# peterrum/deal-and-ceed-on-gpu

Hardware: AMD Instinct MI355X
Metric: BP5 DoFs/sec per CG iter (p=4, ~1e8 DoFs) + % HBM roofline at 1/2/4/8 GPUs (higher is better)
Workload: dtype f64

## Files before the change

### deal-and-ceed-on-gpu_amd/csrc/bp5_device.hip

```cpp
#include "bp5_device.hpp"


extern "C" int bp5_device_count(int *count)
{
  if (!count) return fail(BP5_ERR_INVALID, "null argument");
  int c = 0;
  hipError_t e = hipGetDeviceCount(&c);
  if (e != hipSuccess) { *count = 0; return fail(BP5_ERR_NO_DEVICE, hipGetErrorString(e)); }
  *count = c;
  return BP5_OK;
}
extern "C" int bp5_vec_alloc(size_t n, double **out)
{
  if (!out) return fail(BP5_ERR_INVALID, "null argument");
  HIP_TRY(hipMalloc((void **)out, std::max<size_t>(n, 1) * sizeof(double)));
  HIP_TRY(hipMemset(*out, 0, std::max<size_t>(n, 1) * sizeof(double)));
  HIP_TRY(hipStreamSynchronize(nullptr));
  return BP5_OK;
}
extern "C" int bp5_vec_free(double *v) { HIP_TRY(hipFree(v)); return BP5_OK; }
extern "C" int bp5_copy_h2d(void *dst, const void *src, size_t bytes) { HIP_TRY(hipMemcpy(dst, src, bytes, hipMemcpyHostToDevice)); return BP5_OK; }
extern "C" int bp5_copy_d2h(void *dst, const void *src, size_t bytes) { HIP_TRY(hipMemcpy(dst, src, bytes, hipMemcpyDeviceToHost)); return BP5_OK; }

static void tuning_from_environment(bp5_mf *mf);
// ... 120 lines not shown
    const uint32_t ns = mf->send_off.back();
    if (mf->recv_off.back() != d->n_ghost) { return fail(BP5_ERR_INVALID, "recv ranges must cover the ghost range"); }
    for (uint32_t s = 0; s < ns; ++s)
      if (d->send_indices_host[s] >= d->n_owned) { return fail(BP5_ERR_INVALID, "send index out of owned range"); }
    BP5_TRY(upload(&mf->d_send_idx, d->send_indices_host, ns));
    std::vector<uint8_t> sd(ns);
    for (uint32_t s = 0; s < ns; ++s) sd[s] = mf->h_constrained[d->send_indices_host[s]] ? 1 : 0;
    BP5_TRY(upload(&mf->d_send_dirichlet, sd.data(), sd.size()));
    HIP_TRY(hipMalloc((void **)&mf->d_sendbuf, std::max<size_t>(ns, 1) * sizeof(double)));
    HIP_TRY(hipMalloc((void **)&mf->d_recvbuf, std::max<size_t>(ns, 1) * sizeof(double)));
  } else if (d->n_ghost) { return fail(BP5_ERR_INVALID, "ghosts without a halo plan"); }
  HIP_TRY(hipMalloc((void **)&mf->d_partials, 8 * PARTIAL_STRIDE * sizeof(double)));
  HIP_TRY(hipMalloc((void **)&mf->d_sc, SC_COUNT * sizeof(double)));
  HIP_TRY(hipMalloc((void **)&mf->d_scalar, 8 * sizeof(double)));
  HIP_TRY(hipMalloc((void **)&mf->d_st, ST_COUNT * sizeof(int)));
  HIP_TRY(hipMemset(mf->d_sc, 0, SC_COUNT * sizeof(double)));
  HIP_TRY(hipMemset(mf->d_st, 0, ST_COUNT * sizeof(int)));
  HIP_TRY(hipStreamSynchronize(nullptr));
  HIP_TRY(hipHostMalloc((void **)&mf->h_sc, SC_COUNT * sizeof(double)));
  HIP_TRY(hipHostMalloc((void **)&mf->h_st, ST_COUNT * sizeof(int)));
  HIP_TRY(hipEventCreate(&mf->ev_solve[0]));
  HIP_TRY(hipEventCreate(&mf->ev_solve[1]));
  guard.m = nullptr;
  *out = mf;
  return BP5_OK;
}

extern "C" int bp5_mf_destroy(bp5_mf *mf)
{
  if (!mf) return BP5_OK;
  hipSetDevice(mf->device);
  hipStreamSynchronize(mf->stream);
  void *ptrs[] = {mf->d_constrained_bits, mf->d_l2g, mf->d_constrained, mf->d_send_idx, mf->d_coords, mf->d_tab, mf->d_tab_gauss, mf->d_l2g_padded,
                  mf->d_constraint_mask, mf->d_inv_jac, mf->d_JxW, mf->d_qpoints, mf->d_sendbuf, mf->d_recvbuf, mf->d_partials,
                  mf->d_sc, mf->d_scalar, mf->d_st, mf->ws_base, mf->d_stamps, mf->d_evec, mf->d_scalar_plane, mf->d_gcell, mf->d_hang_mask, mf->d_hang_I, mf->d_send_dirichlet, mf->d_signal, mf->ws_z, mf->wsc_base, mf->hc_base, mf->d_hc_off};
  for (void *p : ptrs) if (p) hipFree(p);
  if (mf->h_sc) hipHostFree(mf->h_sc);
  if (mf->h_st) hipHostFree(mf->h_st);
  for (hipEvent_t e : mf->ev_pool) hipEventDestroy(e);
  for (hipEvent_t e : mf->phase.ev) hipEventDestroy(e);
  for (hipEvent_t e : mf->ev_solve) if (e) hipEventDestroy(e);
  for (hipEvent_t e : mf->ev_halo) if (e) hipEventDestroy(e);
  for (hipEvent_t e : mf->ev_done) if (e) hipEventDestroy(e);
  if (mf->h_done) hipHostFree(mf->h_done);
  if (mf->comm_stream) { hipStreamSynchronize(mf->comm_stream); hipStreamDestroy(mf->comm_stream); }
  for (auto &kv : mf->march_plans) { hipFree(kv.second.team_off); hipFree(kv.second.entries); }
  for (auto &kv : mf->plans) {
    auto &q = kv.second;
    void *pp[] = {q.off, q.dofs, q.sh_dof, q.sh_off, q.sh_slot, q.pos, q.cell_round, q.team_rounds, q.partial, q.cell_off, q.pass_cell, q.pass_off, q.run_off, q.runs, q.gidx, q.packed, q.lattice, q.cell_pos, q.cr_start, q.cr_dof0, q.cr_soff, q.cr_slots, q.cr_tile};
    for (void *x : pp) if (x) hipFree(x);
// ... 1274 lines not shown
}
static void tuning_from_environment(bp5_mf *mf)
{
  mf->tune[BP5_TUNE_LATTICE_INDICES] = env_int("BP5_LATTICE_INDICES", 1) != 0;
  mf->tune[BP5_TUNE_EARLY_GATHER] = env_int("BP5_EARLY_GATHER", 1) != 0;
  mf->tune[BP5_TUNE_COMBINE_SIGNAL] = env_int("BP5_COMBINE_SIGNAL", 0) == 1;
  { const char *e = getenv("BP5_BOUNDARY_FIRST"); mf->tune[BP5_TUNE_BOUNDARY_FIRST] = !(e && !strcmp(e, "launches")); }
  mf->tune[BP5_TUNE_FOLD_SMALL] = env_int("BP5_FOLD_SMALL", 1) != 0;
  { const int u = env_int("BP5_UPDATE_UNROLL", 1); mf->tune[BP5_TUNE_UPDATE_UNROLL] = (u == 2 || u == 4) ? u : 1; }
  mf->tune[BP5_TUNE_UPDATE_FLAT] = env_int("BP5_UPDATE_FLAT", 1) != 0;
  { const int v = env_int("BP5_UPDATE_NT", -1); mf->tune[BP5_TUNE_UPDATE_NT] = v < 0 ? -1 : v != 0; }
  { const int v = env_int("BP5_COMBINE_WG_PER_CU", 16); mf->tune[BP5_TUNE_COMBINE_WG_PER_CU] = (v >= 0 && v <= 32) ? v : 16; }
  mf->tune[BP5_TUNE_INTERIOR_STORES] = env_int("BP5_INTERIOR_STORES", 1) != 0;
  mf->tune[BP5_TUNE_GHOST_COMBINE_ON_COMM] = env_int("BP5_GHOST_COMBINE_ON_COMM", 0) != 0;
  mf->tune[BP5_TUNE_FACE_CARRY] = env_int("BP5_FACE_CARRY", 1) != 0;
}
extern "C" int bp5_mf_set_tuning(bp5_mf *mf, int knob, int value)
{
  if (!mf || knob < 0 || knob >= BP5_TUNE_COUNT) return fail(BP5_ERR_INVALID, "unknown tuning knob");
  switch (knob) {
    case BP5_TUNE_UPDATE_UNROLL:
      if (value != 1 && value != 2 && value != 4) return fail(BP5_ERR_INVALID, "BP5_TUNE_UPDATE_UNROLL: 1, 2 or 4");
      break;
    case BP5_TUNE_UPDATE_NT:
      if (value < -1 || value > 1) return fail(BP5_ERR_INVALID, "BP5_TUNE_UPDATE_NT: -1, 0 or 1");
      break;
    case BP5_TUNE_COMBINE_WG_PER_CU:
      if (value < 0 || value > 32) return fail(BP5_ERR_INVALID, "BP5_TUNE_COMBINE_WG_PER_CU: 0 ... 32");
      break;
    case BP5_TUNE_LATTICE_INDICES:
      if (value != 0 && value != 1) return fail(BP5_ERR_INVALID, "switch: 0 or 1");
      if (value != mf->tune[knob] && mf->plans.count(-block_cpt(mf))) return fail(BP5_ERR_INVALID, "BP5_TUNE_LATTICE_INDICES: the block plan of this handle is already built");
      break;
    default:
      if (value != 0 && value != 1) return fail(BP5_ERR_INVALID, "switch: 0 or 1");
  }
  mf->tune[knob] = value;
  if (knob == BP5_TUNE_BOUNDARY_FIRST && mf->wait_value_ok >= 0) mf->can_wait_value = mf->wait_value_ok == 1 && value != 0;
  return BP5_OK;
}
extern "C" int bp5_mf_get_tuning(const bp5_mf *mf, int knob, int *value)
{
  if (!mf || !value || knob < 0 || knob >= BP5_TUNE_COUNT) return fail(BP5_ERR_INVALID, "unknown tuning knob");
  *value = mf->tune[knob];
// ... 74 lines not shown
  if (mf->overlap_now) HIP_TRY(hipEventRecord(mf->ev_halo[3], cs));
  return BP5_OK;
}
extern "C" int bp5_halo_scatter_add_start(bp5_mf *mf, double *v)
{
  if (!mf || !v) return fail(BP5_ERR_INVALID, "null argument");
  if (mf->neighbors.empty()) return BP5_OK;
  if (!mf->comm) return fail(BP5_ERR_INVALID, "halo exchange needs bp5_mf_set_comm");
  HIP_TRY(hipSetDevice(mf->device));
  BP5_TRY(halo_streams(mf));
  return scatter_exchange(mf, v, overlap_wanted(mf));
}
static int scatter_add_finish(bp5_mf *mf, double *v, FuseState *fuse)
{
  if (mf->overlap_now) HIP_TRY(hipStreamWaitEvent(mf->stream, mf->ev_halo[3], 0));
  for (size_t k = 0; k < mf->neighbors.size(); ++k) {
    const uint32_t sc = mf->send_off[k + 1] - mf->send_off[k];
    if (!sc) continue;
    if (fuse) {
      const uint32_t grid = std::min<uint32_t>((sc + 255) / 256, 1024u / (uint32_t)mf->neighbors.size());
      const uint32_t ng = fuse->ghosts_zeroed ? 0u : mf->n_ghost;
      hipLaunchKernelGGL(unpack_add_dots_kernel, dim3(grid), dim3(256), 0, mf->stream, mf->d_send_idx + mf->send_off[k],
                         mf->d_send_dirichlet + mf->send_off[k], sc, mf->d_recvbuf + mf->send_off[k], v, fuse->r, mf->d_partials,
                         fuse->n_cols, mf->d_st, v + mf->n_owned, const_cast<double *>(fuse->p) + mf->n_owned, ng);
      fuse->n_cols += grid;
      fuse->ghosts_zeroed = true;
    } else
      hipLaunchKernelGGL(unpack_add_kernel, dim3((sc + 255) / 256), dim3(256), 0, mf->stream, mf->d_send_idx + mf->send_off[k], sc,
                         mf->d_recvbuf + mf->send_off[k], v);
    KERNEL_CHECK();
  }
  if (fuse && fuse->ghosts_zeroed) return BP5_OK;
  return bp5_halo_zero_ghosts(mf, v);
}
extern "C" int bp5_halo_scatter_add_finish(bp5_mf *mf, double *v)
{
  if (!mf || !v) return fail(BP5_ERR_INVALID, "null argument");
  if (mf->neighbors.empty()) return BP5_OK;
  if (!mf->comm || !mf->comm_stream) return fail(BP5_ERR_INVALID, "bp5_halo_scatter_add_finish without bp5_halo_scatter_add_start");
  return scatter_add_finish(mf, v, nullptr);
}
// ... 324 lines not shown
  int mark(int k)
  {
    if (!on) return BP5_OK;
    if (used >= 4 * MAX_PROFILED) { on = false; return BP5_OK; }
    while ((size_t)used + 4 > mf->ev_pool.size()) { hipEvent_t e; HIP_TRY(hipEventCreate(&e)); mf->ev_pool.push_back(e); }
    HIP_TRY(hipEventRecord(mf->ev_pool[used + k], mf->stream));
    return BP5_OK;
  }
};

struct SolveState {
  ApplyProfile prof;
  int exchange = EXCHANGE_NONE;
  bool two_parts = false;
  bool gather_in_flight = false;
  bool dst_prezeroed = false, copies_dirichlet = false;
  bool phase_on = false;
  int phase_it = 0;
  uint8_t phase_recorded[bp5_mf::PhaseProfile::MAX_ITERS] = {};
};

static int phase_mark(bp5_mf *mf, SolveState &ss, int k)
{
  if (!ss.phase_on || ss.phase_it >= bp5_mf::PhaseProfile::MAX_ITERS) return BP5_OK;
  HIP_TRY(hipEventRecord(mf->phase.ev[(size_t)ss.phase_it * bp5_mf::PhaseProfile::MARKS + k], mf->stream));
  ss.phase_recorded[ss.phase_it] |= (uint8_t)(1u << k);
  return BP5_OK;
}

static int fused_unsplit(bp5_mf *mf, SolveState &ss, ApplyCall &call, const double *coef, const double *src, double *dst)
// ... 75 lines not shown
  BP5_TRY(phase_mark(mf, ss, 3));
  return scatter_add_finish(mf, dst, call.fuse);
}
static int fused_vmult_distributed(bp5_mf *mf, SolveState &ss, const double *coef, double *src, double *dst, const double *fuse_r, uint32_t *n_cols)
{
  if (ss.gather_in_flight) { ss.gather_in_flight = false; BP5_TRY(bp5_halo_gather_finish(mf, src)); }
  else {
    BP5_TRY(gather_start(mf, src, false));
    BP5_TRY(bp5_halo_gather_finish(mf, src));
  }
  BP5_TRY(phase_mark(mf, ss, 2));
  BP5_TRY(ss.prof.mark(0));
  BP5_TRY(ss.prof.mark(1));
  FuseState fuse;
  fuse.p = src; fuse.r = fuse_r;
  ApplyCall call;
  call.c0 = 0; call.c1 = mf->n_cells; call.overwrite = true;
  call.fuse = &fuse;
  call.exchange = ss.exchange;
  call.two_parts = ss.two_parts;
  if (ss.exchange == EXCHANGE_BOUNDARY_FIRST) BP5_TRY(fused_boundary_first(mf, ss, call, coef, src, dst));
  else if (ss.exchange == EXCHANGE_GHOST_ROWS_FIRST) BP5_TRY(fused_ghost_rows_first(mf, ss, call, coef, src, dst));
  else BP5_TRY(fused_unsplit(mf, ss, call, coef, src, dst));
  *n_cols = fuse.n_cols;
  if (!fuse.ghosts_zeroed) BP5_TRY(bp5_halo_zero_ghosts(mf, src));
  return BP5_OK;
}

static int solver_vmult(bp5_mf *mf, SolveState &ss, const double *coef, double *src, double *dst, bool zero, const double *fuse_r = nullptr,
                        uint32_t *n_cols = nullptr)
{
  ApplyProfile &prof = ss.prof;
  const bool dist = mf->has_neighbors();
  const bool fusing = n_cols != nullptr;
  if (dist && fusing) return fused_vmult_distributed(mf, ss, coef, src, dst, fuse_r, n_cols);
  ApplyCall call;
  call.c0 = 0; call.c1 = mf->n_cells;
  if (dist) {
    BP5_TRY(prof.mark(0));
// ... 281 lines not shown
  const int unroll = mf->tune[BP5_TUNE_UPDATE_UNROLL];
  const int gridu = stream_grid_flat(mf, n, 2 * unroll);
  const bool streaming = mf->tune[BP5_TUNE_UPDATE_NT] != 0;
  auto launch_update = [&](int mode) {
#define BP5_UPD(M, U, ZV, NT) hipLaunchKernelGGL((cgm_update_kernel<M, U, ZV, NT>), dim3(gridu), dim3(VB), 0, s, d, g, h, x, diag, n, mf->d_sc, mf->d_st)
#define BP5_UPD_U(M, ZV, NT) do { if (unroll == 1) BP5_UPD(M, 1, ZV, NT); else if (unroll == 2) BP5_UPD(M, 2, ZV, NT); else BP5_UPD(M, 4, ZV, NT); } while (0)
    if (mode == 0) { BP5_UPD_U(0, false, false); return; }
    if (prezero) { if (mode == 1) BP5_UPD_U(1, true, false); else BP5_UPD_U(2, true, false); return; }
    if (streaming) { if (mode == 1) BP5_UPD_U(1, false, true); else BP5_UPD_U(2, false, true); return; }
    if (mode == 1) BP5_UPD_U(1, false, false); else BP5_UPD_U(2, false, false);
#undef BP5_UPD_U
#undef BP5_UPD
  };
  const bool early_gather_enabled = mf->tune[BP5_TUNE_EARLY_GATHER] != 0;
  const bool early_gather = fused && dist_solve && early_gather_enabled;
  auto gather_under_update = [&](int mode) -> int {
    BP5_TRY(halo_streams(mf));
    const uint32_t ns = mf->send_off.back();
    if (ns) {
      const dim3 gr((ns + 255) / 256), bl(256);
      if (mode == 0) hipLaunchKernelGGL(cgm_pack_updated_kernel<0>, gr, bl, 0, s, mf->d_send_idx, ns, d, g, h, diag, mf->d_sc, mf->d_st, mf->d_sendbuf);
      else hipLaunchKernelGGL(cgm_pack_updated_kernel<1>, gr, bl, 0, s, mf->d_send_idx, ns, d, g, h, diag, mf->d_sc, mf->d_st, mf->d_sendbuf);
      KERNEL_CHECK();
    }
    return gather_exchange(mf, d, true);
  };
  int it = 1;
  for (; it <= prm->max_iter; ++it) {
    const int mode = it == 1 ? 0 : it % 2 == 0 ? 1 : 2;
    BP5_TRY(phase_mark(mf, ss, 0));
    if (early_gather) { BP5_TRY(gather_under_update(mode)); ss.gather_in_flight = true; }
    if (mode != 0) launch_update(mode);
    KERNEL_CHECK();
    BP5_TRY(phase_mark(mf, ss, 1));
    const bool one_launch = fused && !mf->comm;
    if (fused) {
      uint32_t n_cols = 0;
      BP5_TRY(vmult(d, h, g, &n_cols));
      BP5_TRY(phase_mark(mf, ss, 4));
      if (one_launch) hipLaunchKernelGGL(cgm_finalize4_kernel<true>, dim3(1), dim3(FIN4_THREADS), 0, s, mf->d_partials, (int)n_cols, mf->d_sc, mf->d_st);
      else hipLaunchKernelGGL(cgm_finalize4_kernel<false>, dim3(1), dim3(FIN4_THREADS), 0, s, mf->d_partials, (int)n_cols, mf->d_sc, mf->d_st);
    } else {
      BP5_TRY(vmult(d, h, nullptr, nullptr));
      BP5_TRY(phase_mark(mf, ss, 4));
      hipLaunchKernelGGL(cgm_dots_kernel, dim3(grid2), dim3(VB), 0, s, d, g, h, diag, n, mf->d_st, mf->d_partials,
                         fold_small ? (const uint32_t *)mf->d_constrained_bits : (const uint32_t *)nullptr);
      hipLaunchKernelGGL(finalize_kernel<7>, dim3(7), dim3(VB), 0, s, mf->d_partials, grid2, mf->d_sc + SC_R0, mf->d_st);
    }
    KERNEL_CHECK();
    BP5_TRY(phase_mark(mf, ss, 5));
    if (!one_launch) {
      BP5_TRY(bp5_comm_allreduce_sum(mf, mf->d_sc + SC_R0, 7));
      BP5_TRY(phase_mark(mf, ss, 6));
      hipLaunchKernelGGL(cgm_control_kernel, dim3(1), dim3(1), 0, s, mf->d_sc, mf->d_st);
      KERNEL_CHECK();
    } else
      BP5_TRY(phase_mark(mf, ss, 6));
    BP5_TRY(phase_mark(mf, ss, 7));
    if (ss.phase_on) ++ss.phase_it;
    if (check > 0 && it % check == 0 && it < prm->max_iter) {
      BP5_TRY(poll_state(mf));
      if (mf->h_st[ST_DONE]) break;
    }
  }
  if (prm->max_iter > 0) {
    launch_update(1);
    hipLaunchKernelGGL(cgm_control_kernel, dim3(1), dim3(1), 0, s, mf->d_sc, mf->d_st);
    KERNEL_CHECK();
  }
  const int status = solve_finish(mf, ss.prof, fused, op.schedule, !user, res);
// ... 742 lines not shown
```

### deal-and-ceed-on-gpu_amd/csrc/bp5_device.hpp

```cpp
#pragma once
#include "bp5_internal.hpp"
#include "bp5_kernels.hpp"

#include <hip/hip_runtime.h>
#include <rccl/rccl.h>

#include <algorithm>
#include <cmath>
#include <cstdio>
#include <cstdlib>
#include <cstring>
#include <map>
#include <memory>
#include <tuple>
#include <vector>

using namespace bp5;

#define HIP_TRY(expr)                                                                                              \
  do {                                                                                                             \
    hipError_t e_ = (expr);                                                                                        \
    if (e_ != hipSuccess)                                                                                          \
      return fail(e_ == hipErrorNoDevice || e_ == hipErrorInvalidDevice ? BP5_ERR_NO_DEVICE : BP5_ERR_HIP,         \
                  std::string(#expr) + ": " + hipGetErrorString(e_));                                              \
// ... 51 lines not shown
  uint32_t pad = 0;
  std::vector<int> neighbors;
  std::vector<uint32_t> send_off, recv_off;
  double *d_sendbuf = nullptr, *d_recvbuf = nullptr;
  uint8_t *d_send_dirichlet = nullptr;
  bp5_comm *comm = nullptr;
  hipStream_t comm_stream = nullptr;
  hipEvent_t ev_halo[4] = {nullptr, nullptr, nullptr, nullptr};
  int overlap = 2;
  bool overlap_now = false;
  bool cg_fusion = true;
  unsigned long long *d_signal = nullptr;
  uint64_t signal_target = 0;
  int wait_value_ok = -1;
  int can_wait_value = -1;
  int tune[BP5_TUNE_COUNT] = {1, 1, 0, 1, 1, 1, 1, -1, 16, 1, 0, 1};
  bool cell_interiors_first = false;
  double *d_partials = nullptr, *d_sc = nullptr, *d_scalar = nullptr;
  int *d_st = nullptr;
  double *ws_g = nullptr, *ws_d = nullptr, *ws_h = nullptr, *d_evec = nullptr;
  char *ws_base = nullptr;
  double *ws_z = nullptr;
  double *wsc_base = nullptr;
  size_t wsc_cap = 0;
  double *hc_base = nullptr;
  size_t hc_cap = 0;
  uint32_t *d_hc_off = nullptr;
  int *h_done = nullptr;
  hipEvent_t ev_done[3] = {nullptr, nullptr, nullptr};
  unsigned long long *d_stamps = nullptr;
  double *h_sc = nullptr;
  int *h_st = nullptr;
  std::vector<hipEvent_t> ev_pool;
  hipEvent_t ev_solve[2] = {nullptr, nullptr};
// ... 26 lines not shown
    bool covers_all = false;
  };
  std::vector<bool> h_constrained;
  std::vector<uint32_t> h_block_off;
  struct DevMarch { uint32_t *team_off = nullptr, *entries = nullptr; uint32_t n_teams = 0; };
  std::map<int, DevMarch> march_plans;
  std::map<int, DevPlan> plans;
  size_t n_local() const { return (size_t)n_owned + n_ghost; }
  bool has_neighbors() const { return comm && !neighbors.empty(); }
};

struct FuseState {
  const double *p = nullptr, *r = nullptr;
  uint32_t n_cols = 0;
  bool ghosts_zeroed = false;
};
enum VariantFamily { VARIANT_PENCIL, VARIANT_TEAM, VARIANT_MARCH, VARIANT_BLOCK, VARIANT_BLOCK_SIBLING, VARIANT_HANGING_PENCIL, VARIANT_OTHER };
struct VariantInfo {
  VariantFamily family;
  bool atomic_scatter;
  bool shared_by_atomics;
  bool csr_combine;
  bool overwrites;
};
constexpr VariantInfo decode_variant(int v)
{
  const int b = v % 100;
  const VariantFamily f = b <= 6 ? VARIANT_PENCIL : b >= 10 && b <= 14 ? VARIANT_TEAM : b == 56 ? VARIANT_BLOCK : b >= 48 && b <= 63 ? VARIANT_BLOCK_SIBLING
                        : b >= 70 && b <= 72 ? VARIANT_MARCH : b == 90 ? VARIANT_HANGING_PENCIL : VARIANT_OTHER;
  return {f, v >= 100, b == 54 || b == 55, b == 48, v < 100 && (f == VARIANT_TEAM || f == VARIANT_BLOCK || f == VARIANT_BLOCK_SIBLING)};
// ... 767 lines not shown
```

### deal-and-ceed-on-gpu_amd/csrc/bp5_kernels.hpp

```cpp
#pragma once
#include <hip/hip_runtime.h>
#include <stdint.h>
#include <type_traits>

namespace bp5 {

template <int n>
struct ShapeArg {
  double N[n * n];
  double D[n * n];
};

enum : int {
  BLK_AFFINE = 1024, BLK_SINGLE = 2048, BLK_STAMPS = 4096, BLK_SEQ = 8192, BLK_RUNS = 16384, BLK_NTM = 32768, BLK_PACK = 262144,
  BLK_STAGE = 524288, BLK_FUSE = 1048576, BLK_HANG = 2097152, BLK_LDSADD = 4194304, BLK_HELM = 8388608, BLK_LATT = 16777216,
  BLK_ROLL = 67108864, BLK_CARRY = 268435456,
  BLK_F32M = 536870912,
  BLK_MASS = 1073741824,
  BLK_DEFAULT = BLK_SINGLE | BLK_SEQ | BLK_RUNS | BLK_PACK
};
enum : int {
  PEN_INTERIOR_STORES = 32,
  PEN_NT_LOADS = 256,
  PEN_FULL_OCCUPANCY = 512
// ... 3197 lines not shown
    buf[halo_message_pos(off, n_nb, i, blockIdx.y, gridDim.y)] = *g;
    *g = 0.0;
  }
}
static __global__ void unpack_add_components_kernel(const uint32_t *idx, uint32_t n, const double *buf, double *v, size_t ld)
{
  const uint32_t i = blockIdx.x * blockDim.x + threadIdx.x;
  if (i < n) v[blockIdx.y * ld + idx[i]] += buf[(size_t)blockIdx.y * n + i];
}
static __global__ void zero_ghosts_components_kernel(double *ghosts, uint32_t n, size_t ld)
{
  const uint32_t i = blockIdx.x * blockDim.x + threadIdx.x;
  if (i < n) ghosts[blockIdx.y * ld + i] = 0.0;
}

static __global__ void __launch_bounds__(256) unpack_add_dots_kernel(const uint32_t *idx, const uint8_t *dirichlet, uint32_t n, const double *buf, double *v,
                                                                     const double *r, double *partials, uint32_t col0, const int *state,
                                                                     double *ghosts_a, double *ghosts_b, uint32_t n_ghost)
{
  if (state[0]) return;
  for (uint32_t i = blockIdx.x * 256u + threadIdx.x; i < n_ghost; i += gridDim.x * 256u) { ghosts_a[i] = 0.0; ghosts_b[i] = 0.0; }
  __shared__ double red[2][4];
  double dvv = 0.0, drv = 0.0;
  for (uint32_t i = blockIdx.x * 256u + threadIdx.x; i < n; i += gridDim.x * 256u) {
    if (dirichlet[i]) continue;
    const uint32_t g = idx[i];
    const double c = buf[i], vo = v[g], vn = vo + c;
    v[g] = vn;
    dvv += vn * vn - vo * vo;
    if (r) drv += r[g] * c;
  }
#pragma unroll
  for (int off = 32; off > 0; off >>= 1) { dvv += __shfl_down(dvv, off, 64); drv += __shfl_down(drv, off, 64); }
  if ((threadIdx.x & 63) == 0) { red[0][threadIdx.x >> 6] = dvv; red[1][threadIdx.x >> 6] = drv; }
  __syncthreads();
  if (threadIdx.x < 7) {
    const int t = threadIdx.x;
    const double svv = (red[0][0] + red[0][1]) + (red[0][2] + red[0][3]), srv = (red[1][0] + red[1][1]) + (red[1][2] + red[1][3]);
    partials[t * PARTIAL_STRIDE + col0 + blockIdx.x] = (t == 1 || t == 5) ? svv : (t == 2 || t == 4) ? srv : 0.0;
  }
}

constexpr int VB = 256;
constexpr int MAXBLK = 2048;

template <int MODE>
__global__ void __launch_bounds__(VB) vec_kernel(double *y, const double *x, double s, double a, size_t n)
{
  const size_t stride = (size_t)gridDim.x * VB * 2;
  for (size_t i = ((size_t)blockIdx.x * VB + threadIdx.x) * 2; i < n; i += stride) {
    if (i + 1 < n) {
      double2 yv = *reinterpret_cast<double2 *>(y + i);
      double2 xv = MODE ? *reinterpret_cast<const double2 *>(x + i) : double2{0, 0};
      if (MODE == 0) { yv.x = s; yv.y = s; }
      if (MODE == 1) { yv.x += a * xv.x; yv.y += a * xv.y; }
// ... 276 lines not shown
          if (MODE != 0) *reinterpret_cast<double2 *>(r + i) = rv[u];
        }
        if (touch_x) {
          if constexpr (NTX) __builtin_nontemporal_store(bp5_d2u{xv[u].x, xv[u].y}, reinterpret_cast<bp5_d2u *>(x + i));
          else *reinterpret_cast<double2 *>(x + i) = xv[u];
        }
        if constexpr (ZV) { if (MODE != 0 && !done) *reinterpret_cast<double2 *>(v + i) = double2{0.0, 0.0}; }
      } else {
        if (touch_rp) { p[i] = pv[u].x; if (MODE != 0) r[i] = rv[u].x; }
        if (touch_x) x[i] = xv[u].x;
        if constexpr (ZV) { if (MODE != 0 && !done) v[i] = 0.0; }
      }
    }
  }
}
template <int MODE>
__global__ void __launch_bounds__(256) cgm_pack_updated_kernel(const uint32_t *idx, uint32_t n, const double *p, const double *r, const double *v,
                                                             const double *diag, const double *sc, const int *st, double *buf)
{
  const uint32_t i = blockIdx.x * 256u + threadIdx.x;
  if (i >= n) return;
  const uint32_t g = idx[i];
  double pi = p[g];
  if (!st[ST_DONE]) {
    double ri = r[g], xi = 0.0;
    const double vi = MODE != 0 ? v[g] : 0.0;
    cgm_update_one<MODE>(pi, ri, vi, xi, diag ? diag[g] : 1.0, false, false, sc[SC_ALPHA], sc[SC_BETA], 0.0);
  }
  buf[i] = pi;
}

static __global__ void __launch_bounds__(VB) cgm_dots_kernel(const double *p, const double *r, double *v, const double *diag, size_t n,
                                                     const int *st, double *partials, const uint32_t *cbits)
{
  if (st[ST_DONE]) return;
  double acc[7] = {0, 0, 0, 0, 0, 0, 0};
  auto one = [&](double pi, double ri, double vi, double di) {
    acc[0] += pi * vi; acc[1] += vi * vi; acc[2] += ri * vi; acc[3] += ri * ri;
    acc[4] += ri * di * vi; acc[5] += vi * di * vi; acc[6] += ri * di * ri;
  };
  const size_t stride = (size_t)gridDim.x * VB * 2;
  for (size_t i = ((size_t)blockIdx.x * VB + threadIdx.x) * 2; i < n; i += stride) {
// ... 4 lines not shown
      if (cb) {
        if (cb & 1u) vv.x = pv.x;
        if (cb & 2u) vv.y = pv.y;
        *reinterpret_cast<double2 *>(v + i) = vv;
      }
      one(pv.x, rv.x, vv.x, diag ? diag[i] : 1.0);
      one(pv.y, rv.y, vv.y, diag ? diag[i + 1] : 1.0);
    } else {
      double vi = v[i];
      if (cb & 1u) { vi = p[i]; v[i] = vi; }
      one(p[i], r[i], vi, diag ? diag[i] : 1.0);
    }
  }
  block_reduce_store<7>(acc, partials);
}
static __global__ void cgm_control_kernel(double *sc, int *st);
__device__ __forceinline__ void cgm_control_step(double *sc, int *st)
{
  if (st[ST_DONE]) { st[ST_PENDING] = 0; return; }
  const double *R = sc + SC_R0;
  if (!(R[0] == R[0]) || R[0] == 0.0) { st[ST_BREAKDOWN] = 1; st[ST_DONE] = 1; return; }
  sc[SC_ALPHA_OLD] = sc[SC_ALPHA];
  sc[SC_BETA_OLD] = sc[SC_BETA];
  const double alpha = R[6] / R[0];
  sc[SC_ALPHA] = alpha;
  const double r2 = R[3] + 2.0 * alpha * R[2] + alpha * alpha * R[1];
  const double res = sqrt(r2 > 0.0 ? r2 : 0.0);
  sc[SC_RES] = res;
  const int it = ++st[ST_ITER];
  if (res <= sc[SC_TOL] || it >= st[ST_MAXIT]) { st[ST_DONE] = 1; st[ST_PENDING] = 1; return; }
  sc[SC_BETA] = alpha * (R[4] + alpha * R[5]) / R[6];
}
constexpr int FIN4_THREADS = 1024;
template <bool CONTROL>
__global__ void __launch_bounds__(FIN4_THREADS) cgm_finalize4_kernel(const double *partials, int nblk, double *sc, int *st)
{
  if (st[ST_DONE]) {
    if (CONTROL && threadIdx.x == 0) cgm_control_step(sc, st);
    return;
  }
  __shared__ double red[16];
  const int wave = threadIdx.x >> 6, lane = threadIdx.x & 63;
  const int k = wave >> 2, l = ((wave & 3) << 6) | lane;
  const double *row = partials + k * PARTIAL_STRIDE;
  double s0 = 0.0, s1 = 0.0, s2 = 0.0, s3 = 0.0;
  for (int i = l; i < nblk; i += 1024) {
    const double a0 = row[i], a1 = i + 256 < nblk ? row[i + 256] : 0.0, a2 = i + 512 < nblk ? row[i + 512] : 0.0, a3 = i + 768 < nblk ? row[i + 768] : 0.0;
    s0 += a0; s1 += a1; s2 += a2; s3 += a3;
  }
  double s = (s0 + s1) + (s2 + s3);
#pragma unroll
  for (int off = 32; off > 0; off >>= 1) s += __shfl_down(s, off, 64);
  if (lane == 0) red[wave] = s;
  __syncthreads();
  double *out = sc + SC_R0;
  if (threadIdx.x < 4) {
    const int r = threadIdx.x;
    const double t = (red[4 * r] + red[4 * r + 1]) + (red[4 * r + 2] + red[4 * r + 3]);
    out[r] = t;
    if (r == 1) out[5] = t;
    if (r == 2) out[4] = t;
    if (r == 3) out[6] = t;
  }
  if constexpr (CONTROL) {
    __syncthreads();
    if (threadIdx.x == 0) cgm_control_step(sc, st);
  }
}

static __global__ void cgm_control_kernel(double *sc, int *st) { cgm_control_step(sc, st); }

static __global__ void __launch_bounds__(VB) cgm_init_kernel(const double *b, double *x, double *r, double *p, double *v, const double *diag, size_t n,
                                                     double *partials, bool zero_v)
{
  double acc[2] = {0.0, 0.0};
  const size_t stride = (size_t)gridDim.x * VB;
  for (size_t i = (size_t)blockIdx.x * VB + threadIdx.x; i < n; i += stride) {
    const double ri = -b[i], di = diag ? diag[i] : 1.0;
// ... 685 lines not shown
```

### deal-and-ceed-on-gpu_amd/matrix_free.py

```python
import ctypes as C

import numpy as np

from . import _lib
from ._lib import BP5Error, CG_MERGED, CG_PLAIN, COEF_ONE, QUAD_GAUSS


def _torch():
    import torch
    return torch


def _ptr(t, n_min=0):
    torch = _torch()
    if t is None:
        return None
    if not (isinstance(t, torch.Tensor) and t.is_cuda and t.dtype == torch.float64 and t.is_contiguous()):
        raise BP5Error(1, "expected a contiguous float64 CUDA tensor")
    if t.numel() < n_min:
        raise BP5Error(1, f"vector has {t.numel()} entries, need {n_min}")
    return C.c_void_p(t.data_ptr())


class Communicator:
# ... 110 lines not shown
            raise BP5Error(1, f"metric precision must be 'float64' or 'float32', not {precision!r}")
        _lib.check(_lib.lib().bp5_mf_set_metric_precision(self.handle, self.METRIC_PRECISION[precision]))

    def get_metric_precision(self):
        v = C.c_int()
        _lib.check(_lib.lib().bp5_mf_get_metric_precision(self.handle, C.byref(v)))
        return "float32" if v.value == 1 else "float64"

    def set_block_workgroups(self, n):
        _lib.check(_lib.lib().bp5_mf_set_block_workgroups(self.handle, int(n)))

    def set_streaming(self, policy):
        _lib.check(_lib.lib().bp5_mf_set_streaming(self.handle, int(policy)))

    TUNE = {"lattice_indices": 0, "early_gather": 1, "combine_signal": 2, "boundary_first": 3, "fold_small": 4, "update_unroll": 5,
            "update_flat": 6, "update_nt": 7, "combine_wg_per_cu": 8, "interior_stores": 9, "ghost_combine_on_comm": 10, "face_carry": 11}

    def set_tuning(self, knob, value):
        _lib.check(_lib.lib().bp5_mf_set_tuning(self.handle, int(self.TUNE.get(knob, knob)), int(value)))

    def get_tuning(self, knob):
        v = C.c_int()
        _lib.check(_lib.lib().bp5_mf_get_tuning(self.handle, int(self.TUNE.get(knob, knob)), C.byref(v)))
        return v.value

    def wait_value_available(self):
        v = C.c_int()
        _lib.check(_lib.lib().bp5_mf_wait_value_available(self.handle, C.byref(v)))
        return bool(v.value)

    def block_plan_info(self):
# ... 610 lines not shown
```

### include/bp5.h

```cpp
#ifndef BP5_H
#define BP5_H

#include <stddef.h>
#include <stdint.h>

#ifdef __cplusplus
extern "C" {
#endif

enum {
  BP5_OK = 0,
  BP5_ERR_INVALID = 1,
  BP5_ERR_HIP = 2,
  BP5_ERR_NO_DEVICE = 3,
  BP5_ERR_RCCL = 4,
  BP5_ERR_UNSUPPORTED = 5,
  BP5_ERR_BREAKDOWN = 6,
  BP5_ERR_NO_CONVERGENCE = 7
};
const char *bp5_strerror(int status);
const char *bp5_last_error(void);

enum { BP5_QUAD_GAUSS = 0,
       BP5_QUAD_GLL = 1,
// ... 112 lines not shown

int bp5_apply(bp5_mf *mf, const double *coef, const double *src, double *dst, int zero_dst);
int bp5_apply_cells(bp5_mf *mf, const double *coef, const double *src, double *dst, uint32_t cell_begin,
                    uint32_t cell_end);
int bp5_copy_constrained(bp5_mf *mf, const double *src, double *dst);
int bp5_set_constrained(bp5_mf *mf, double value, double *dst);

#define BP5_MAX_COMPONENTS 8
int bp5_apply_components(bp5_mf *mf, const double *coef, int n_components, size_t ld, const double *src, double *dst, int zero_dst);

int bp5_mf_set_apply_variant(bp5_mf *mf, int variant);
int bp5_mf_set_block_workgroups(bp5_mf *mf, int max_workgroups);
int bp5_mf_set_streaming(bp5_mf *mf, int policy);
enum { BP5_TUNE_LATTICE_INDICES = 0, BP5_TUNE_EARLY_GATHER = 1, BP5_TUNE_COMBINE_SIGNAL = 2, BP5_TUNE_BOUNDARY_FIRST = 3,
       BP5_TUNE_FOLD_SMALL = 4, BP5_TUNE_UPDATE_UNROLL = 5, BP5_TUNE_UPDATE_FLAT = 6, BP5_TUNE_UPDATE_NT = 7, BP5_TUNE_COMBINE_WG_PER_CU = 8,
       BP5_TUNE_INTERIOR_STORES = 9, BP5_TUNE_GHOST_COMBINE_ON_COMM = 10, BP5_TUNE_FACE_CARRY = 11, BP5_TUNE_COUNT = 12 };
int bp5_mf_set_tuning(bp5_mf *mf, int knob, int value);
int bp5_mf_get_tuning(const bp5_mf *mf, int knob, int *value);
int bp5_mf_wait_value_available(bp5_mf *mf, int *available);
int bp5_mf_block_plan_info(bp5_mf *mf, uint32_t *n_blocks, uint32_t *max_runs, int *packed_indices);
int bp5_mf_block_plan_lattice(bp5_mf *mf, uint32_t *n_lattice_blocks);
int bp5_mf_block_plan_carry(bp5_mf *mf, uint32_t *n_faces, uint32_t *n_shared, uint32_t *n_shared_last_launch);
int bp5_mf_get_apply_variant(bp5_mf *mf, int *effective);

int bp5_compute_diagonal(bp5_mf *mf, const double *coef, double *diag, int invert);

int bp5_assemble_rhs(bp5_mf *mf, double *b);
int bp5_l2_norm_solution(bp5_mf *mf, const double *u, double *result_host);

int bp5_vec_fill(bp5_mf *mf, double *v, double value, size_t n);
int bp5_vec_axpy(bp5_mf *mf, double *y, double a, const double *x, size_t n);
// ... 137 lines not shown
```

Baseline: 28.19 billion.

## Fuse CG control step into halo pack kernel and partial sums into unpack tail

```diff
diff --git a/deal-and-ceed-on-gpu_amd/csrc/bp5_device.hip b/deal-and-ceed-on-gpu_amd/csrc/bp5_device.hip
--- a/deal-and-ceed-on-gpu_amd/csrc/bp5_device.hip
+++ b/deal-and-ceed-on-gpu_amd/csrc/bp5_device.hip
@@ -158,8 +158,14 @@
   HIP_TRY(hipMalloc((void **)&mf->d_sc, SC_COUNT * sizeof(double)));
   HIP_TRY(hipMalloc((void **)&mf->d_scalar, 8 * sizeof(double)));
   HIP_TRY(hipMalloc((void **)&mf->d_st, ST_COUNT * sizeof(int)));
+  HIP_TRY(hipMalloc((void **)&mf->d_sc_alt, SC_COUNT * sizeof(double)));
+  HIP_TRY(hipMalloc((void **)&mf->d_st_alt, ST_COUNT * sizeof(int)));
+  HIP_TRY(hipMalloc((void **)&mf->d_tail_count, sizeof(unsigned)));
   HIP_TRY(hipMemset(mf->d_sc, 0, SC_COUNT * sizeof(double)));
   HIP_TRY(hipMemset(mf->d_st, 0, ST_COUNT * sizeof(int)));
+  HIP_TRY(hipMemset(mf->d_sc_alt, 0, SC_COUNT * sizeof(double)));
+  HIP_TRY(hipMemset(mf->d_st_alt, 0, ST_COUNT * sizeof(int)));
+  HIP_TRY(hipMemset(mf->d_tail_count, 0, sizeof(unsigned)));
   HIP_TRY(hipStreamSynchronize(nullptr));
   HIP_TRY(hipHostMalloc((void **)&mf->h_sc, SC_COUNT * sizeof(double)));
   HIP_TRY(hipHostMalloc((void **)&mf->h_st, ST_COUNT * sizeof(int)));
@@ -177,7 +183,8 @@
   hipStreamSynchronize(mf->stream);
   void *ptrs[] = {mf->d_constrained_bits, mf->d_l2g, mf->d_constrained, mf->d_send_idx, mf->d_coords, mf->d_tab, mf->d_tab_gauss, mf->d_l2g_padded,
                   mf->d_constraint_mask, mf->d_inv_jac, mf->d_JxW, mf->d_qpoints, mf->d_sendbuf, mf->d_recvbuf, mf->d_partials,
-                  mf->d_sc, mf->d_scalar, mf->d_st, mf->ws_base, mf->d_stamps, mf->d_evec, mf->d_scalar_plane, mf->d_gcell, mf->d_hang_mask, mf->d_hang_I, mf->d_send_dirichlet, mf->d_signal, mf->ws_z, mf->wsc_base, mf->hc_base, mf->d_hc_off};
+                  mf->d_sc, mf->d_scalar, mf->d_st, mf->ws_base, mf->d_stamps, mf->d_evec, mf->d_scalar_plane, mf->d_gcell, mf->d_hang_mask, mf->d_hang_I, mf->d_send_dirichlet, mf->d_signal, mf->ws_z, mf->wsc_base, mf->hc_base, mf->d_hc_off,
+                  mf->d_sc_alt, mf->d_st_alt, mf->d_tail_count};
   for (void *p : ptrs) if (p) hipFree(p);
   if (mf->h_sc) hipHostFree(mf->h_sc);
   if (mf->h_st) hipHostFree(mf->h_st);
@@ -1482,6 +1489,7 @@
   mf->tune[BP5_TUNE_INTERIOR_STORES] = env_int("BP5_INTERIOR_STORES", 1) != 0;
   mf->tune[BP5_TUNE_GHOST_COMBINE_ON_COMM] = env_int("BP5_GHOST_COMBINE_ON_COMM", 0) != 0;
   mf->tune[BP5_TUNE_FACE_CARRY] = env_int("BP5_FACE_CARRY", 1) != 0;
+  { const int v = env_int("BP5_TAIL_FUSION", 1); mf->tune[BP5_TUNE_TAIL_FUSION] = (v == 0 || v == 2) ? v : 1; }
 }
 extern "C" int bp5_mf_set_tuning(bp5_mf *mf, int knob, int value)
 {
@@ -1496,6 +1504,9 @@
     case BP5_TUNE_COMBINE_WG_PER_CU:
       if (value < 0 || value > 32) return fail(BP5_ERR_INVALID, "BP5_TUNE_COMBINE_WG_PER_CU: 0 ... 32");
       break;
+    case BP5_TUNE_TAIL_FUSION:
+      if (value < 0 || value > 2) return fail(BP5_ERR_INVALID, "BP5_TUNE_TAIL_FUSION: 0, 1 or 2");
+      break;
     case BP5_TUNE_LATTICE_INDICES:
       if (value != 0 && value != 1) return fail(BP5_ERR_INVALID, "switch: 0 or 1");
       if (value != mf->tune[knob] && mf->plans.count(-block_cpt(mf))) return fail(BP5_ERR_INVALID, "BP5_TUNE_LATTICE_INDICES: the block plan of this handle is already built");
@@ -1600,17 +1611,22 @@
 static int scatter_add_finish(bp5_mf *mf, double *v, FuseState *fuse)
 {
   if (mf->overlap_now) HIP_TRY(hipStreamWaitEvent(mf->stream, mf->ev_halo[3], 0));
+  size_t k_last = mf->neighbors.size();
+  for (size_t k = 0; k < mf->neighbors.size(); ++k) if (mf->send_off[k + 1] > mf->send_off[k]) k_last = k;
   for (size_t k = 0; k < mf->neighbors.size(); ++k) {
     const uint32_t sc = mf->send_off[k + 1] - mf->send_off[k];
     if (!sc) continue;
     if (fuse) {
       const uint32_t grid = std::min<uint32_t>((sc + 255) / 256, 1024u / (uint32_t)mf->neighbors.size());
       const uint32_t ng = fuse->ghosts_zeroed ? 0u : mf->n_ghost;
+      const bool tail = fuse->tail_out && k == k_last;
       hipLaunchKernelGGL(unpack_add_dots_kernel, dim3(grid), dim3(256), 0, mf->stream, mf->d_send_idx + mf->send_off[k],
                          mf->d_send_dirichlet + mf->send_off[k], sc, mf->d_recvbuf + mf->send_off[k], v, fuse->r, mf->d_partials,
-                         fuse->n_cols, mf->d_st, v + mf->n_owned, const_cast<double *>(fuse->p) + mf->n_owned, ng);
+                         fuse->n_cols, mf->d_st, v + mf->n_owned, const_cast<double *>(fuse->p) + mf->n_owned, ng,
+                         tail ? mf->d_tail_count : (unsigned *)nullptr, fuse->n_cols + grid, fuse->tail_out);
       fuse->n_cols += grid;
       fuse->ghosts_zeroed = true;
+      fuse->tail_summed = tail;
     } else
       hipLaunchKernelGGL(unpack_add_kernel, dim3((sc + 255) / 256), dim3(256), 0, mf->stream, mf->d_send_idx + mf->send_off[k], sc,
                          mf->d_recvbuf + mf->send_off[k], v);
@@ -1965,6 +1981,7 @@
   int exchange = EXCHANGE_NONE;
   bool two_parts = false;
   bool gather_in_flight = false;
+  bool tail_sums = false, tail_summed = false;
   bool dst_prezeroed = false, copies_dirichlet = false;
   bool phase_on = false;
   int phase_it = 0;
@@ -2070,6 +2087,7 @@
   BP5_TRY(ss.prof.mark(1));
   FuseState fuse;
   fuse.p = src; fuse.r = fuse_r;
+  if (ss.tail_sums) fuse.tail_out = mf->d_sc + SC_R0;
   ApplyCall call;
   call.c0 = 0; call.c1 = mf->n_cells; call.overwrite = true;
   call.fuse = &fuse;
@@ -2079,6 +2097,7 @@
   else if (ss.exchange == EXCHANGE_GHOST_ROWS_FIRST) BP5_TRY(fused_ghost_rows_first(mf, ss, call, coef, src, dst));
   else BP5_TRY(fused_unsplit(mf, ss, call, coef, src, dst));
   *n_cols = fuse.n_cols;
+  ss.tail_summed = fuse.tail_summed;
   if (!fuse.ghosts_zeroed) BP5_TRY(bp5_halo_zero_ghosts(mf, src));
   return BP5_OK;
 }
@@ -2390,13 +2409,23 @@
   };
   const bool early_gather_enabled = mf->tune[BP5_TUNE_EARLY_GATHER] != 0;
   const bool early_gather = fused && dist_solve && early_gather_enabled;
+  const int tail_fusion = fused && dist_solve && mf->comm ? mf->tune[BP5_TUNE_TAIL_FUSION] : 0;
+  const bool step_in_pack = tail_fusion >= 1 && early_gather && mf->send_off.back() > 0;
+  bool step_pending = false;
+  ss.tail_sums = tail_fusion == 2;
   auto gather_under_update = [&](int mode) -> int {
     BP5_TRY(halo_streams(mf));
     const uint32_t ns = mf->send_off.back();
     if (ns) {
       const dim3 gr((ns + 255) / 256), bl(256);
-      if (mode == 0) hipLaunchKernelGGL(cgm_pack_updated_kernel<0>, gr, bl, 0, s, mf->d_send_idx, ns, d, g, h, diag, mf->d_sc, mf->d_st, mf->d_sendbuf);
-      else hipLaunchKernelGGL(cgm_pack_updated_kernel<1>, gr, bl, 0, s, mf->d_send_idx, ns, d, g, h, diag, mf->d_sc, mf->d_st, mf->d_sendbuf);
+      if (mode == 0) hipLaunchKernelGGL((cgm_pack_updated_kernel<0, false>), gr, bl, 0, s, mf->d_send_idx, ns, d, g, h, diag, mf->d_sc, mf->d_st, mf->d_sendbuf, (double *)nullptr, (int *)nullptr);
+      else if (!step_pending) hipLaunchKernelGGL((cgm_pack_updated_kernel<1, false>), gr, bl, 0, s, mf->d_send_idx, ns, d, g, h, diag, mf->d_sc, mf->d_st, mf->d_sendbuf, (double *)nullptr, (int *)nullptr);
+      else {
+        hipLaunchKernelGGL((cgm_pack_updated_kernel<1, true>), gr, bl, 0, s, mf->d_send_idx, ns, d, g, h, diag, mf->d_sc, mf->d_st, mf->d_sendbuf, mf->d_sc_alt, mf->d_st_alt);
+        std::swap(mf->d_sc, mf->d_sc_alt);
+        std::swap(mf->d_st, mf->d_st_alt);
+        step_pending = false;
+      }
       KERNEL_CHECK();
     }
     return gather_exchange(mf, d, true);
@@ -2412,10 +2441,12 @@
     const bool one_launch = fused && !mf->comm;
     if (fused) {
       uint32_t n_cols = 0;
+      ss.tail_summed = false;
       BP5_TRY(vmult(d, h, g, &n_cols));
       BP5_TRY(phase_mark(mf, ss, 4));
       if (one_launch) hipLaunchKernelGGL(cgm_finalize4_kernel<true>, dim3(1), dim3(FIN4_THREADS), 0, s, mf->d_partials, (int)n_cols, mf->d_sc, mf->d_st);
-      else hipLaunchKernelGGL(cgm_finalize4_kernel<false>, dim3(1), dim3(FIN4_THREADS), 0, s, mf->d_partials, (int)n_cols, mf->d_sc, mf->d_st);
+      else if (!ss.tail_summed)
+        hipLaunchKernelGGL(cgm_finalize4_kernel<false>, dim3(1), dim3(FIN4_THREADS), 0, s, mf->d_partials, (int)n_cols, mf->d_sc, mf->d_st);
     } else {
       BP5_TRY(vmult(d, h, nullptr, nullptr));
       BP5_TRY(phase_mark(mf, ss, 4));
@@ -2428,8 +2459,12 @@
     if (!one_launch) {
       BP5_TRY(bp5_comm_allreduce_sum(mf, mf->d_sc + SC_R0, 7));
       BP5_TRY(phase_mark(mf, ss, 6));
-      hipLaunchKernelGGL(cgm_control_kernel, dim3(1), dim3(1), 0, s, mf->d_sc, mf->d_st);
-      KERNEL_CHECK();
+      const bool looks = check > 0 && it % check == 0;
+      if (step_in_pack && it < prm->max_iter && !looks) step_pending = true;
+      else {
+        hipLaunchKernelGGL(cgm_control_kernel, dim3(1), dim3(1), 0, s, mf->d_sc, mf->d_st);
+        KERNEL_CHECK();
+      }
     } else
       BP5_TRY(phase_mark(mf, ss, 6));
     BP5_TRY(phase_mark(mf, ss, 7));
diff --git a/deal-and-ceed-on-gpu_amd/csrc/bp5_device.hpp b/deal-and-ceed-on-gpu_amd/csrc/bp5_device.hpp
--- a/deal-and-ceed-on-gpu_amd/csrc/bp5_device.hpp
+++ b/deal-and-ceed-on-gpu_amd/csrc/bp5_device.hpp
@@ -89,10 +89,13 @@
   uint64_t signal_target = 0;
   int wait_value_ok = -1;
   int can_wait_value = -1;
-  int tune[BP5_TUNE_COUNT] = {1, 1, 0, 1, 1, 1, 1, -1, 16, 1, 0, 1};
+  int tune[BP5_TUNE_COUNT] = {1, 1, 0, 1, 1, 1, 1, -1, 16, 1, 0, 1, 1};
   bool cell_interiors_first = false;
   double *d_partials = nullptr, *d_sc = nullptr, *d_scalar = nullptr;
   int *d_st = nullptr;
+  double *d_sc_alt = nullptr;
+  int *d_st_alt = nullptr;
+  unsigned *d_tail_count = nullptr;
   double *ws_g = nullptr, *ws_d = nullptr, *ws_h = nullptr, *d_evec = nullptr;
   char *ws_base = nullptr;
   double *ws_z = nullptr;
@@ -149,6 +152,8 @@
   const double *p = nullptr, *r = nullptr;
   uint32_t n_cols = 0;
   bool ghosts_zeroed = false;
+  double *tail_out = nullptr;
+  bool tail_summed = false;
 };
 enum VariantFamily { VARIANT_PENCIL, VARIANT_TEAM, VARIANT_MARCH, VARIANT_BLOCK, VARIANT_BLOCK_SIBLING, VARIANT_HANGING_PENCIL, VARIANT_OTHER };
 struct VariantInfo {
diff --git a/deal-and-ceed-on-gpu_amd/csrc/bp5_kernels.hpp b/deal-and-ceed-on-gpu_amd/csrc/bp5_kernels.hpp
--- a/deal-and-ceed-on-gpu_amd/csrc/bp5_kernels.hpp
+++ b/deal-and-ceed-on-gpu_amd/csrc/bp5_kernels.hpp
@@ -3235,9 +3235,46 @@
   if (i < n) ghosts[blockIdx.y * ld + i] = 0.0;
 }
 
+template <int THREADS>
+__device__ __forceinline__ void cgm_sum_rows(const double *partials, int nblk, double *out)
+{
+  static_assert(THREADS % 64 == 0 && THREADS >= 256 && 1024 % THREADS == 0, "whole waves, at least the four roles of a row at once");
+  __shared__ double red[16];
+  constexpr int NR = 1024 / THREADS;
+  const int lane = threadIdx.x & 63, wave = threadIdx.x >> 6;
+  const int l = ((wave & 3) << 6) | lane;
+  const double *row0 = partials + (wave >> 2) * PARTIAL_STRIDE;
+  double acc[NR][4] = {};
+  for (int i = l; i < nblk; i += 1024) {
+#pragma unroll
+    for (int j = 0; j < NR; ++j) {
+      const double *row = row0 + j * (THREADS / 256) * PARTIAL_STRIDE;
+      const double a0 = row[i], a1 = i + 256 < nblk ? row[i + 256] : 0.0, a2 = i + 512 < nblk ? row[i + 512] : 0.0, a3 = i + 768 < nblk ? row[i + 768] : 0.0;
+      acc[j][0] += a0; acc[j][1] += a1; acc[j][2] += a2; acc[j][3] += a3;
+    }
+  }
+#pragma unroll
+  for (int j = 0; j < NR; ++j) {
+    double s = (acc[j][0] + acc[j][1]) + (acc[j][2] + acc[j][3]);
+#pragma unroll
+    for (int off = 32; off > 0; off >>= 1) s += __shfl_down(s, off, 64);
+    if (lane == 0) red[wave + j * (THREADS / 64)] = s;
+  }
+  __syncthreads();
+  if (threadIdx.x < 4) {
+    const int r = threadIdx.x;
+    const double t = (red[4 * r] + red[4 * r + 1]) + (red[4 * r + 2] + red[4 * r + 3]);
+    out[r] = t;
+    if (r == 1) out[5] = t;
+    if (r == 2) out[4] = t;
+    if (r == 3) out[6] = t;
+  }
+}
+
 static __global__ void __launch_bounds__(256) unpack_add_dots_kernel(const uint32_t *idx, const uint8_t *dirichlet, uint32_t n, const double *buf, double *v,
                                                                      const double *r, double *partials, uint32_t col0, const int *state,
-                                                                     double *ghosts_a, double *ghosts_b, uint32_t n_ghost)
+                                                                     double *ghosts_a, double *ghosts_b, uint32_t n_ghost, unsigned *tail_count,
+                                                                     uint32_t tail_cols, double *tail_out)
 {
   if (state[0]) return;
   for (uint32_t i = blockIdx.x * 256u + threadIdx.x; i < n_ghost; i += gridDim.x * 256u) { ghosts_a[i] = 0.0; ghosts_b[i] = 0.0; }
@@ -3260,6 +3297,18 @@
     const double svv = (red[0][0] + red[0][1]) + (red[0][2] + red[0][3]), srv = (red[1][0] + red[1][1]) + (red[1][2] + red[1][3]);
     partials[t * PARTIAL_STRIDE + col0 + blockIdx.x] = (t == 1 || t == 5) ? svv : (t == 2 || t == 4) ? srv : 0.0;
   }
+  if (!tail_count) return;
+  __shared__ int last;
+  __syncthreads();
+  if (threadIdx.x == 0) {
+    __builtin_amdgcn_fence(__ATOMIC_RELEASE, "agent");
+    last = __hip_atomic_fetch_add(tail_count, 1u, __ATOMIC_RELAXED, __HIP_MEMORY_SCOPE_AGENT) == gridDim.x - 1u;
+  }
+  __syncthreads();
+  if (!last) return;
+  __builtin_amdgcn_fence(__ATOMIC_ACQUIRE, "agent");
+  if (threadIdx.x == 0) __hip_atomic_store(tail_count, 0u, __ATOMIC_RELAXED, __HIP_MEMORY_SCOPE_AGENT);
+  cgm_sum_rows<256>(partials, (int)tail_cols, tail_out);
 }
 
 constexpr int VB = 256;
@@ -3566,18 +3615,60 @@
     }
   }
 }
-template <int MODE>
+struct CgmStep {
+  double alpha, beta, alpha_old, beta_old, res;
+  int done, iter, pending, breakdown;
+};
+__device__ __forceinline__ CgmStep cgm_control_eval(const double *sc, const int *st)
+{
+  CgmStep n{sc[SC_ALPHA], sc[SC_BETA], sc[SC_ALPHA_OLD], sc[SC_BETA_OLD], sc[SC_RES], st[ST_DONE], st[ST_ITER], st[ST_PENDING], st[ST_BREAKDOWN]};
+  if (n.done) { n.pending = 0; return n; }
+  const double *R = sc + SC_R0;
+  if (!(R[0] == R[0]) || R[0] == 0.0) { n.breakdown = 1; n.done = 1; return n; }
+  n.alpha_old = n.alpha;
+  n.beta_old = n.beta;
+  const double alpha = R[6] / R[0];
+  n.alpha = alpha;
+  const double r2 = R[3] + 2.0 * alpha * R[2] + alpha * alpha * R[1];
+  const double res = sqrt(r2 > 0.0 ? r2 : 0.0);
+  n.res = res;
+  const int it = ++n.iter;
+  if (res <= sc[SC_TOL] || it >= st[ST_MAXIT]) { n.done = 1; n.pending = 1; return n; }
+  n.beta = alpha * (R[4] + alpha * R[5]) / R[6];
+  return n;
+}
+__device__ __forceinline__ void cgm_control_store(const CgmStep &n, const double *sc, const int *st, double *sc_to, int *st_to)
+{
+  if (sc_to != sc) {
+    for (int k = 0; k < SC_R0; ++k) sc_to[k] = sc[k];
+    for (int k = 0; k < ST_COUNT; ++k) st_to[k] = st[k];
+  }
+  sc_to[SC_ALPHA] = n.alpha; sc_to[SC_BETA] = n.beta; sc_to[SC_ALPHA_OLD] = n.alpha_old; sc_to[SC_BETA_OLD] = n.beta_old; sc_to[SC_RES] = n.res;
+  st_to[ST_DONE] = n.done; st_to[ST_ITER] = n.iter; st_to[ST_PENDING] = n.pending; st_to[ST_BREAKDOWN] = n.breakdown;
+}
+__device__ __forceinline__ void cgm_control_step(double *sc, int *st) { cgm_control_store(cgm_control_eval(sc, st), sc, st, sc, st); }
+template <int MODE, bool STEP = false>
 __global__ void __launch_bounds__(256) cgm_pack_updated_kernel(const uint32_t *idx, uint32_t n, const double *p, const double *r, const double *v,
-                                                             const double *diag, const double *sc, const int *st, double *buf)
+                                                             const double *diag, const double *sc, const int *st, double *buf, double *sc_to,
+                                                             int *st_to)
 {
   const uint32_t i = blockIdx.x * 256u + threadIdx.x;
+  bool done;
+  double alpha, beta;
+  if constexpr (STEP) {
+    const CgmStep now = cgm_control_eval(sc, st);
+    if (i == 0) cgm_control_store(now, sc, st, sc_to, st_to);
+    done = now.done; alpha = now.alpha; beta = now.beta;
+  } else {
+    done = st[ST_DONE]; alpha = sc[SC_ALPHA]; beta = sc[SC_BETA];
+  }
   if (i >= n) return;
   const uint32_t g = idx[i];
   double pi = p[g];
-  if (!st[ST_DONE]) {
+  if (!done) {
     double ri = r[g], xi = 0.0;
     const double vi = MODE != 0 ? v[g] : 0.0;
-    cgm_update_one<MODE>(pi, ri, vi, xi, diag ? diag[g] : 1.0, false, false, sc[SC_ALPHA], sc[SC_BETA], 0.0);
+    cgm_update_one<MODE>(pi, ri, vi, xi, diag ? diag[g] : 1.0, false, false, alpha, beta, 0.0);
   }
   buf[i] = pi;
 }
@@ -3612,23 +3703,6 @@
   }
   block_reduce_store<7>(acc, partials);
 }
-static __global__ void cgm_control_kernel(double *sc, int *st);
-__device__ __forceinline__ void cgm_control_step(double *sc, int *st)
-{
-  if (st[ST_DONE]) { st[ST_PENDING] = 0; return; }
-  const double *R = sc + SC_R0;
-  if (!(R[0] == R[0]) || R[0] == 0.0) { st[ST_BREAKDOWN] = 1; st[ST_DONE] = 1; return; }
-  sc[SC_ALPHA_OLD] = sc[SC_ALPHA];
-  sc[SC_BETA_OLD] = sc[SC_BETA];
-  const double alpha = R[6] / R[0];
-  sc[SC_ALPHA] = alpha;
-  const double r2 = R[3] + 2.0 * alpha * R[2] + alpha * alpha * R[1];
-  const double res = sqrt(r2 > 0.0 ? r2 : 0.0);
-  sc[SC_RES] = res;
-  const int it = ++st[ST_ITER];
-  if (res <= sc[SC_TOL] || it >= st[ST_MAXIT]) { st[ST_DONE] = 1; st[ST_PENDING] = 1; return; }
-  sc[SC_BETA] = alpha * (R[4] + alpha * R[5]) / R[6];
-}
 constexpr int FIN4_THREADS = 1024;
 template <bool CONTROL>
 __global__ void __launch_bounds__(FIN4_THREADS) cgm_finalize4_kernel(const double *partials, int nblk, double *sc, int *st)
@@ -3637,29 +3711,7 @@
     if (CONTROL && threadIdx.x == 0) cgm_control_step(sc, st);
     return;
   }
-  __shared__ double red[16];
-  const int wave = threadIdx.x >> 6, lane = threadIdx.x & 63;
-  const int k = wave >> 2, l = ((wave & 3) << 6) | lane;
-  const double *row = partials + k * PARTIAL_STRIDE;
-  double s0 = 0.0, s1 = 0.0, s2 = 0.0, s3 = 0.0;
-  for (int i = l; i < nblk; i += 1024) {
-    const double a0 = row[i], a1 = i + 256 < nblk ? row[i + 256] : 0.0, a2 = i + 512 < nblk ? row[i + 512] : 0.0, a3 = i + 768 < nblk ? row[i + 768] : 0.0;
-    s0 += a0; s1 += a1; s2 += a2; s3 += a3;
-  }
-  double s = (s0 + s1) + (s2 + s3);
-#pragma unroll
-  for (int off = 32; off > 0; off >>= 1) s += __shfl_down(s, off, 64);
-  if (lane == 0) red[wave] = s;
-  __syncthreads();
-  double *out = sc + SC_R0;
-  if (threadIdx.x < 4) {
-    const int r = threadIdx.x;
-    const double t = (red[4 * r] + red[4 * r + 1]) + (red[4 * r + 2] + red[4 * r + 3]);
-    out[r] = t;
-    if (r == 1) out[5] = t;
-    if (r == 2) out[4] = t;
-    if (r == 3) out[6] = t;
-  }
+  cgm_sum_rows<FIN4_THREADS>(partials, nblk, sc + SC_R0);
   if constexpr (CONTROL) {
     __syncthreads();
     if (threadIdx.x == 0) cgm_control_step(sc, st);
diff --git a/deal-and-ceed-on-gpu_amd/matrix_free.py b/deal-and-ceed-on-gpu_amd/matrix_free.py
--- a/deal-and-ceed-on-gpu_amd/matrix_free.py
+++ b/deal-and-ceed-on-gpu_amd/matrix_free.py
@@ -148,7 +148,8 @@
         _lib.check(_lib.lib().bp5_mf_set_streaming(self.handle, int(policy)))
 
     TUNE = {"lattice_indices": 0, "early_gather": 1, "combine_signal": 2, "boundary_first": 3, "fold_small": 4, "update_unroll": 5,
-            "update_flat": 6, "update_nt": 7, "combine_wg_per_cu": 8, "interior_stores": 9, "ghost_combine_on_comm": 10, "face_carry": 11}
+            "update_flat": 6, "update_nt": 7, "combine_wg_per_cu": 8, "interior_stores": 9, "ghost_combine_on_comm": 10, "face_carry": 11,
+            "tail_fusion": 12}
 
     def set_tuning(self, knob, value):
         _lib.check(_lib.lib().bp5_mf_set_tuning(self.handle, int(self.TUNE.get(knob, knob)), int(value)))
diff --git a/include/bp5.h b/include/bp5.h
--- a/include/bp5.h
+++ b/include/bp5.h
@@ -150,7 +150,7 @@
 int bp5_mf_set_streaming(bp5_mf *mf, int policy);
 enum { BP5_TUNE_LATTICE_INDICES = 0, BP5_TUNE_EARLY_GATHER = 1, BP5_TUNE_COMBINE_SIGNAL = 2, BP5_TUNE_BOUNDARY_FIRST = 3,
        BP5_TUNE_FOLD_SMALL = 4, BP5_TUNE_UPDATE_UNROLL = 5, BP5_TUNE_UPDATE_FLAT = 6, BP5_TUNE_UPDATE_NT = 7, BP5_TUNE_COMBINE_WG_PER_CU = 8,
-       BP5_TUNE_INTERIOR_STORES = 9, BP5_TUNE_GHOST_COMBINE_ON_COMM = 10, BP5_TUNE_FACE_CARRY = 11, BP5_TUNE_COUNT = 12 };
+       BP5_TUNE_INTERIOR_STORES = 9, BP5_TUNE_GHOST_COMBINE_ON_COMM = 10, BP5_TUNE_FACE_CARRY = 11, BP5_TUNE_TAIL_FUSION = 12, BP5_TUNE_COUNT = 13 };
 int bp5_mf_set_tuning(bp5_mf *mf, int knob, int value);
 int bp5_mf_get_tuning(const bp5_mf *mf, int knob, int *value);
 int bp5_mf_wait_value_available(bp5_mf *mf, int *available);
```

Result: no change. 28.23 billion, median of 2 (+0.1%).
